# tdavchev/DESIRE

Hardware: AMD Instinct MI355X
Metric: agent-trajectory-samples/sec (K=20, T_pred=40) (higher is better)
Workload: dtype f32; 1 GPU; BASELINE configs[1]: SDD-like synthetic windows, 32 agent slots/window, K=20, T_obs=8/T_pred=40, H=128, L=128, fp32, posterior CVAE, IOC 1 refinement, social grid 4x4, scene grid 64x64x32; 512 windows/step/GPU; windows_per_gpu=512, rows_per_gpu=327680, parallelism=scene-sharded x1

## Files before the change

desire_amd/csrc/api.hip:

```cpp
#include "ctx.h"

#include <cmath>
#include <cstdio>
#include <cstdlib>
#include <cstring>

static thread_local std::string g_err;
int desire_fail(int code, const std::string& msg) { g_err = msg; return code; }

extern "C" const char* desire_last_error(void) { return g_err.c_str(); }
extern "C" int desire_version(void) { return 5; }
extern "C" int desire_dims_size(void) { return (int)sizeof(desire_dims); }
#ifndef DESIRE_SRC_HASH
#define DESIRE_SRC_HASH "unstamped"
#endif
extern "C" const char* desire_build_hash(void) { return DESIRE_SRC_HASH; }

int desire_upload(desire_ctx* h, const std::string& name, const std::vector<float>& v) {
    const size_t bytes = v.size() * sizeof(float);
    const DevBuf* b = h->dev.find(name.c_str());
    if (!b || b->bytes != bytes) {
        h->dev.release(name.c_str());
        if (h->dev.ensure(name.c_str(), bytes)) return -1;
    }
// ... 76 lines not shown
        return fail(DESIRE_ERR_ARG, "mno must divide 32 or be a multiple of 32 up to 256 (above 128: inference, step-wise IOC)");
    if (d.mno > 128 && d.bf16 == 1) return fail(DESIRE_ERR_ARG, "more than 128 agents per scene run the fp32 step-wise IOC (bf16 = 0, 2 or 3)");
    if (d.H != 16 && d.H != 32 && d.H != 64 && d.H != 128 && d.H != 256)
        return fail(DESIRE_ERR_ARG, "H must be 16, 32 (run zero-padded on the 64-wide tile), 64, 128 or 256");

    if (d.L % 8 || d.L < 8) return fail(DESIRE_ERR_ARG, "L must be a positive multiple of 8");
    if (d.C != 32 || d.E_v != 16) return fail(DESIRE_ERR_ARG, "C=32 and E_v=16 are the instantiated IOC widths in this round");
    if (d.n_scenes < 1 || d.K < 1 || d.T_obs < 1 || d.T_pred < 1 || d.n_grids < 1 || d.iters < 1 || d.Gh < 1 || d.Gw < 1)
        return fail(DESIRE_ERR_ARG, "sizes must be >= 1");
    if (d.grid_size < 1 || d.grid_size > 6) return fail(DESIRE_ERR_ARG, "grid_size must be 1..6 (6 x 6 = the paper's 36 bins)");
    if (d.grid_size > 4 && d.H == 256) return fail(DESIRE_ERR_ARG, "grid_size 5..6 needs H <= 128 (LDS budget of the IOC tile)");
    if (d.bf16 < 0 || d.bf16 > 3)
        return fail(DESIRE_ERR_ARG, "bf16 must be 0 (fp32 operands), 1 (bf16 operands), 2 (split-bf16 operands: hi + lo, three products) or 3 (three "
                                    "bf16 pieces, six products: fp32-class accuracy)");
    if (d.bn_mode < 0 || d.bn_mode > 2) return fail(DESIRE_ERR_ARG, "bn_mode must be 0 (frozen statistics), 1 (per-object statistics) or 2 (whole-batch statistics)");
    if (d.bn_mode && d.bf16 == 1) return fail(DESIRE_ERR_ARG, "batch statistics (bn_mode 1 / 2) run on fp32 operands (bf16 = 0 or 2)");
    if (d.bin_mode != 0 && d.bin_mode != 1) return fail(DESIRE_ERR_ARG, "bin_mode must be 0 (rectangular) or 1 (log-polar)");
    if (d.bin_mode == 1 && (d.grid_size < 3 || !(d.nb_h > 0.f) || !(d.nb_w > d.nb_h)))
        return fail(DESIRE_ERR_ARG, "log-polar bins: grid_size >= 3 and 0 < nb_h (inner radius) < nb_w (outer radius)");
    if (!(d.nb_w > 0.f) || !(d.nb_h > 0.f)) return fail(DESIRE_ERR_ARG, "nb_w/nb_h must be > 0");
    if (d.ref_compat != 0 && d.ref_compat != 1) return fail(DESIRE_ERR_ARG, "ref_compat must be 0 or 1");
    if (int rc = check_options(d)) return rc;
    if (d.ref_compat) {
        if (d.K != 1 || !d.posterior || d.bn_mode != 1 || d.bf16 || d.n_dec < 1 || d.H != 2 * d.T_obs || d.T_pred != d.T_obs)
            return fail(DESIRE_ERR_ARG, "ref_compat (the reference graph as written, model/model.py:116-311) needs K = 1 (one eps per object, "
                                        ":262-263), posterior = 1, bn_mode = 1, bf16 = 0, H == 2*T_obs (:286-289), T_pred == T_obs and n_dec >= 1 (:280 runs 7)");
    } else if (d.n_dec != 0) return fail(DESIRE_ERR_ARG, "n_dec belongs to ref_compat (0 otherwise)");
    return 0;
}

}

extern "C" int desire_set_option(desire_handle* h, const char* name, int32_t value) {
    if (!h || !name) return fail(DESIRE_ERR_ARG, "null argument");
    desire_dims d = h->d;
    const std::string nm(name);
    if (nm == "ioc_form") d.ioc_form = value;
    else if (nm == "ioc_split") d.ioc_split = value;
    else if (nm == "train_fp32_mask") d.train_fp32_mask = value;
    else if (nm == "flags") d.flags = value;
    else if (nm == "compact_host_counts") {
        h->cp_host_counts = value != 0;
        h->cp_pending = false; h->cp_enc = false;
        return DESIRE_OK;
    }
    else if (nm == "scene_grad") {
        if (value != 0 && value != 1) return fail(DESIRE_ERR_ARG, "scene_grad must be 0 or 1");
        h->scene_grad = value != 0;
        return scene_grad_on(h) && h->training ? scene_grad_setup(h) : DESIRE_OK;
    }
    else if (nm == "compact_min_rows") {
        if (value < 0) return fail(DESIRE_ERR_ARG, "compact_min_rows must be >= 0");
        h->ci_min_rows = value;
        return DESIRE_OK;
    }
    else return fail(DESIRE_ERR_ARG, "unknown option: " + nm + " (ioc_form, ioc_split, train_fp32_mask, flags, compact_min_rows, compact_host_counts, scene_grad)");
    if (int rc = check_options(d)) return rc;
    if (((d.flags ^ h->d.flags) & (DESIRE_FLAG_COMPACT_ROWS | DESIRE_FLAG_COMPACT_IOC)) ||
        ((d.flags & DESIRE_FLAG_COMPACT_IOC) && (d.ioc_form != h->d.ioc_form || d.train_fp32_mask != h->d.train_fp32_mask)))
        h->cp_pending = h->cp_enc = false;
    h->d = d;
    return DESIRE_OK;
}

extern "C" int desire_create(const desire_dims* dims, desire_handle** out) {
    if (!dims || !out) return fail(DESIRE_ERR_ARG, "null argument");
    if (int rc = check_dims(*dims)) return rc;
    int ndev = 0;
    if (hipGetDeviceCount(&ndev) != hipSuccess || ndev < 1)
        return fail(DESIRE_ERR_NODEV, "no HIP device: libdesire_hip has no CPU path");
    int dev = 0;
    HIPCHK(hipGetDevice(&dev));
    hipDeviceProp_t prop;
    HIPCHK(hipGetDeviceProperties(&prop, dev));
    if (std::strncmp(prop.gcnArchName, "gfx950", 6) != 0)
        return fail(DESIRE_ERR_NODEV, std::string("device is ") + prop.gcnArchName + ", kernels are built for gfx950 only");
    desire_ctx* h = new desire_ctx();
    h->d = *dims;
    h->Hl = dims->H;
    if (dims->H < 64) h->d.H = 64;
    h->A = dims->n_scenes * dims->mno;
    h->R = h->A * dims->K;
    h->V = dims->S * dims->S;
    h->B = dims->grid_size * dims->grid_size;
    h->E = dims->E_v + dims->C + h->d.H;
    pack::weight_shapes(h->d, h->d.H, h->V, h->B, h->want);
    pack::weight_shapes(h->d, h->Hl, h->V, h->B, h->want_user);
    if (h->Hl != h->d.H) embeddings(h);
    const desire_dims& d = h->d;
// ... 213 lines not shown
```

desire_amd/csrc/api_forward.hip:

```cpp
#include "ctx.h"

#include <cmath>
#include <cstdio>
#include <cstdlib>
#include <cstring>

bool compact_rows(const desire_ctx* h) { return (h->d.flags & DESIRE_FLAG_COMPACT_ROWS) != 0; }
bool compact_ioc(const desire_ctx* h) { return (h->d.flags & DESIRE_FLAG_COMPACT_IOC) && ioc_plan(h).fwd != IocFwd::STEPWISE; }
ClassLayout class_layout(const desire_ctx* h, bool pad, const int* counts) {
    const desire_dims& d = h->d;
    ClassLayout L;
    int cand[6], nc = 0;
    for (int m : {8, 10, 16, 32, 64, 96}) if (m < d.mno && (m != 10 || pad)) cand[nc++] = m;
    for (int i = nc > 3 ? nc - 3 : 0; i < nc; ++i) L.m[L.n++] = cand[i];
    L.m[L.n++] = d.mno;
    for (int i = L.n; i < 4; ++i) L.m[i] = d.mno;
    for (int c = 0; c < L.n; ++c) {
        IocView& v = L.c[c];
        v.cls = c; v.mno = L.m[c]; v.n_scenes = counts ? counts[c] : d.n_scenes;
        v.gpt = (v.mno <= 32 && 32 % v.mno) ? 32 / v.mno : 0; v.ngrp = v.n_scenes * d.K;
        v.R = v.gpt ? (long)((v.ngrp + v.gpt - 1) / v.gpt) * 32 : (long)v.ngrp * v.mno;
        v.agent_off = L.agents; v.row_off = L.rows; v.win_off = L.wins;
        L.agents += (size_t)v.n_scenes * v.mno; L.rows += (size_t)v.R; L.wins += (size_t)v.n_scenes;
    }
// ... 192 lines not shown
    const bool dyn = compact && compact_dyn(h);
    const int32_t* dynP = dyn ? Wt<const int32_t>(h, "cp_count") : nullptr;
    h->cp_last = compact;
    if (compact) {
        if (int rc = compact_wait(h, s)) return rc;
        int P = h->A;
        if (!dyn) { if (int rc = present_count(h, &P)) return rc; }
        h->cp_P = dyn ? -1 : P;
        R = P * d.K; mno = P;
        const size_t RT2 = (size_t)h->R * d.T_pred * 2;
        if (P == 0) {
            launch_fill_f32(W(h, "Y0"), RT2, 0.f, s); launch_fill_f32(dev_Yhat, RT2, 0.f, s);
            HIPCHK(hipGetLastError());
            return DESIRE_OK;
        }
        const int32_t* amap = Wt<const int32_t>(h, "cp_amap");
        Timer t(h, s, "compact_gather");
        if (!h->cp_enc) {
            launch_gather_agents(W(h, "HxHy"), W(h, "cp_HxHy"), amap, P, 2 * H, s, dynP);
            launch_gather_agents(W(h, "p_last"), W(h, "cp_plast"), amap, P, 2, s, dynP);
            if (d.posterior) launch_gather_agents(W(h, "params"), W(h, "cp_params"), amap, P, 2 * d.L, s, dynP);
        }
        HxS = W(h, "cp_HxHy"); plS = W(h, "cp_plast"); Yout = W(h, "cp_Y0");
    }
    if (compact) { Timer t(h, s, "reparam"); launch_reparam_c(W(h, "cp_params"), dev_eps, W(h, "z"), Wt<const int32_t>(h, "cp_amap"), mno, d.K, d.mno, d.L, d.posterior, s, dynP); }
    else { Timer t(h, s, "reparam"); launch_reparam(W(h, "params"), dev_eps, W(h, "z"), R, d.L, d.K, d.mno, d.posterior, s); }
    auto normd = [&](const char* layer, float* x, int P, int C, int sig) { batch_stats_act(h, layer, x, R, P, C, sig, s); };
    GemmArgs g{};
    g.A = W(h, "z"); g.lda = d.L; g.M = R; g.K = d.L; g.Bp = D4(h, "vae_dec/deconv1/W"); g.G = d.L / 8;
    g.NT = 64; g.out = W(h, "d1"); g.ldo = 2048; g.N = 2048;
    g.p0 = D(h, "vae_dec/deconv1/scale"); g.p1 = D(h, "vae_dec/deconv1/shift"); g.chmod = 128;
    int hintS = 0;
    if (dyn) hintS = count_hint(h);
    g.dyn = DynCount{dynP, d.K, hintS}; g.M_hint = hintS * d.K;
    const bool x6gen = ((d.bf16 == 3 && !h->training) || (d.bf16 == 2 && (!h->training || (train_x3_mask(h) & 8)))) && d.bn_mode == 0 && !d.ref_compat;
    if (d.bf16 == 1 && d.L <= 512 && !(d.L & 15)) { g.Bp = D4(h, "vae_dec/deconv1/W16"); Timer t(h, s, "deconv1"); launch_deconv1_bf16(g, s); }
    else if (x6gen && rows_x6_supported(d.L, 64)) { g.Bp = D4(h, "vae_dec/deconv1/W6"); Timer t(h, s, "deconv1"); launch_deconv1_x6(g, s); }
    else if (d.bn_mode != 0) {
        Timer t(h, s, "deconv1"); launch_gemm_rows(g, EPI_NONE, s);
        normd("vae_dec/deconv1", W(h, "d1"), 16, 128, 0);
    }
    else { Timer t(h, s, "deconv1"); launch_gemm_rows(g, EPI_SCALE_SHIFT_ELU, s); }
    ConvArgs c{};
    c.n = R; c.dyn = DynCount{dynP, d.K, hintS};
    const bool pobn = d.bn_mode != 0;
    if (pobn) c.mode = 3;
    c.in = W(h, "d1"); c.out = W(h, "d2"); c.Wp = D4(h, "vae_dec/deconv2/W");
    c.scale = D(h, "vae_dec/deconv2/scale"); c.shift = D(h, "vae_dec/deconv2/shift");
    if (d.bf16 == 1) { c.Wp = D4(h, "vae_dec/deconv2/W16"); Timer t(h, s, "deconv2"); launch_deconv2_bf16(c, s); }
    else if (x6gen) { c.Wp = D4(h, "vae_dec/deconv2/W6"); Timer t(h, s, "deconv2"); launch_deconv2_x6(c, s, (h->training && (d.flags & DESIRE_FLAG_TRAIN_FWD_3P)) ? 2 : 3); }
    else { Timer t(h, s, "deconv2"); launch_deconv2(c, s);
           if (pobn) normd("vae_dec/deconv2", W(h, "d2"), 64, 64, 0); }
    c.in = W(h, "d2"); c.out = W(h, "d3"); c.Wp = D4(h, "vae_dec/deconv3/W");
    c.scale = D(h, "vae_dec/deconv3/scale"); c.shift = D(h, "vae_dec/deconv3/shift");
    const bool fuse34 = d.bf16 == 1 && !(d.flags & DESIRE_FLAG_NO_FUSE34);
    if (fuse34) {
        c.Wp = D4(h, "vae_dec/deconv3/W16"); c.w_raw = D(h, "vae_dec/deconv4/W16"); c.out = W(h, "xhat");
        Timer t(h, s, "deconv34");
        launch_deconv34_bf16(c, D(h, "vae_dec/deconv4/scale"), D(h, "vae_dec/deconv4/shift"), s);
    } else {
        if (d.bf16 == 1) { c.Wp = D4(h, "vae_dec/deconv3/W16"); Timer t(h, s, "deconv3"); launch_deconv3_bf16(c, s); }
        else if (x6gen) { c.Wp = D4(h, "vae_dec/deconv3/W6"); Timer t(h, s, "deconv3"); launch_deconv3_x6(c, s, (h->training && (d.flags & DESIRE_FLAG_TRAIN_FWD_3P)) ? 2 : 3); }
        else { Timer t(h, s, "deconv3"); launch_deconv3(c, s);
               if (pobn) normd("vae_dec/deconv3", W(h, "d3"), 256, 32, 0); }
        c.in = W(h, "d3"); c.out = W(h, "xhat"); c.w_raw = D(h, "vae_dec/deconv4/raw");
        c.scale = D(h, "vae_dec/deconv4/scale"); c.shift = D(h, "vae_dec/deconv4/shift");
        { Timer t(h, s, "deconv4"); launch_deconv4(c, s);
          if (pobn) normd("vae_dec/deconv4", W(h, "xhat"), 1024, 1, 1); }
    }
    MaskArgs m{};
    m.xhat = W(h, "xhat"); m.R = R; m.V = h->V; m.H = H; m.Hl = h->Hl; m.K = d.K; m.mno = mno;
    m.Wp = D4(h, "mask/W"); m.bias = D(h, "mask/b"); m.Hx = HxS; m.ldhx = 2 * H; m.xz = W(h, "xz");
    m.dyn = DynCount{dynP, 1, hintS};
    if (h->training) m.sv_p = W(h, "mask_sv_p");
    if (d.bf16 == 1) { m.Wp = D4(h, "mask/W16"); Timer t(h, s, "mask_fc"); launch_mask_bf16(m, s); }
    else if (x6gen && (H == 64 || H == 128) && h->V % 128 == 0) { m.Wp = D4(h, "mask/W6"); Timer t(h, s, "mask_fc"); launch_mask_x6(m, s); }
    else { Timer t(h, s, "mask_fc"); launch_mask(m, s); }
    DecArgs a{};
    a.xz = W(h, "xz"); a.Hx = HxS; a.ldhx = 2 * H; a.p_last = plS;
    a.R = R; a.K = d.K; a.mno = mno; a.H = H; a.T = d.T_pred;
    a.Wxg = D4(h, "dec/Wxg"); a.Wxc = D4(h, "dec/Wxc"); a.Whg = D4(h, "dec/Whg"); a.Whc = D4(h, "dec/Whc");
    a.b_g = D(h, "dec/gb"); a.b_c = D(h, "dec/cb"); a.w_head = D(h, "head/w"); a.b_head = D(h, "head/b");
    a.Y = Yout; a.hdump = nullptr; a.dyn = DynCount{dynP, 1, hintS};
    if (d.ref_compat) { a.T = d.n_dec; a.hdump = W(h, "dec_states"); }
    if (h->training) { a.hdump = W(h, "dec_sv_h"); a.sv_r = W(h, "dec_sv_r"); a.sv_u = W(h, "dec_sv_u"); a.sv_c = W(h, "dec_sv_c"); }
    if (d.bf16 == 1) {
        a.Whg = D4(h, "dec/Whg16"); a.Whc = D4(h, "dec/Whc16");
        Timer t(h, s, "decoder"); launch_decoder_bf16(a, s);
    } else
    if (x6gen && decoder_x6_supported(H)) {
        a.Whg = D4(h, "dec/Whg6"); a.Whc = D4(h, "dec/Whc6");
        Timer t(h, s, "decoder"); launch_decoder_x6(a, s, (h->training && (d.flags & DESIRE_FLAG_TRAIN_FWD_3P)) ? 2 : 3);
    } else
    { Timer t(h, s, "decoder"); launch_decoder(a, s); }
    if (d.ref_compat)
        launch_copy_cols(dev_Yhat, W(h, "dec_states"), (size_t)R * d.n_dec, h->Hl, H, s);
    else if (compact) {
        Timer t(h, s, "compact_scatter");
        const size_t RT2 = (size_t)h->R * d.T_pred * 2;
        launch_fill_f32(W(h, "Y0"), RT2, 0.f, s); launch_fill_f32(dev_Yhat, RT2, 0.f, s);
        launch_scatter_rows(Yout, W(h, "Y0"), dev_Yhat, Wt<const int32_t>(h, "cp_amap"), mno, d.K, d.mno, d.T_pred * 2, s, dynP);
    } else
        launch_copy_f32(dev_Yhat, W(h, "Y0"), (size_t)R * d.T_pred * 2, s);
    HIPCHK(hipGetLastError());
    return DESIRE_OK;
}

int ioc_cluster_exchange(desire_ctx* h, size_t n_groups, bool reset_err, hipStream_t s) {
    if (int rc = ws_ensure(h, {{"hex", (size_t)2 * h->R * h->d.H * sizeof(float)}, {"grp_cnt", ((size_t)h->R / 32 + 1) * sizeof(int)}, {"ioc_err", sizeof(int)}})) return rc;
    HIPCHK(hipMemsetAsync(W(h, "grp_cnt"), 0, n_groups * sizeof(int), s));
    if (reset_err) HIPCHK(hipMemsetAsync(W(h, "ioc_err"), 0, sizeof(int), s));
    return DESIRE_OK;
}
int ioc_cluster_check(desire_ctx* h, hipStream_t s, const char* what) {
    int err = 0;
    HIPCHK(hipMemcpyAsync(&err, W(h, "ioc_err"), sizeof(int), hipMemcpyDeviceToHost, s));
    HIPCHK(hipStreamSynchronize(s));
    return err ? fail(DESIRE_ERR_HIP, std::string(what) + " hand-off timed out (workgroups of a group were not co-resident)") : DESIRE_OK;
}
#ifdef DESIRE_IOC_TIMING
void ioc_timing_report(const long long* dbg, const char* const* names, int n, hipStream_t s) {
    long long host[16];
    (void)hipStreamSynchronize(s); (void)hipMemcpy(host, dbg, n * sizeof(long long), hipMemcpyDeviceToHost);
    long long tot = 0; for (int k = 0; k < n; ++k) tot += host[k];
    for (int k = 0; k < n; ++k) fprintf(stderr, "[ioc timing] %-45s %12lld cyc  %5.1f%%\n", names[k], host[k], 100.0 * host[k] / (double)tot);
}
#endif

static int ioc_core(desire_handle* h, const IocView& v, hipStream_t s) {
    const desire_dims& d = h->d;
    if (h->training && d.bf16 == 1) return fail(DESIRE_ERR_STATE, "bf16 operands are inference-only");
    IocArgs a{};
    a.Y = v.Y; a.score = v.score; a.Hx = v.Hx; a.ldhx = 2 * d.H; a.p_last = v.p_last; a.valid = v.valid;
    a.R = (int)v.R; a.K = d.K; a.mno = v.mno; a.H = d.H; a.T = d.T_pred; a.iters = d.iters;
    a.C = d.C; a.Gh = d.Gh; a.Gw = d.Gw; a.E_v = d.E_v; a.G = d.grid_size; a.nb_w = d.nb_w; a.nb_h = d.nb_h;
    a.grids = h->grids; a.grid_of_scene = v.gos; a.bin_tab = d.bin_mode == 1 ? W(h, "bin_tab") : nullptr;
    a.w_vel = D(h, "ioc/vel_w"); a.b_vel = D(h, "ioc/vel_b");
    a.Wsoc = D4(h, "ioc/Wsoc"); a.b_soc = D(h, "ioc/soc_b"); a.Wsoc_c = D4(h, "ioc/Wsoc_c");
    a.Wg = D4(h, "ioc/Wg"); a.Wc = D4(h, "ioc/Wc"); a.b_g = D(h, "ioc/gb"); a.b_c = D(h, "ioc/cb");
    a.w_score = D(h, "ioc/score_w"); a.b_score = D(h, "ioc/score_b");
    a.Wreg = D4(h, "ioc/Wreg"); a.b_reg = D(h, "ioc/reg_b"); a.NTreg = (2 * d.T_pred + 31) / 32;
    a.variant = d.ioc_form; a.gpt = v.gpt; a.ngrp = v.ngrp; a.dyn = DynCount{v.dynN, 1, 0};
    const IocPlan p = ioc_plan(d, h->training, v.mno, v.gpt, v.R, [&](int n) { return ioc_bin_split_capacity(a, n); });
    if (!p.fp32_weights()) { a.Wsoc = D4(h, "ioc/Wsoc16"); a.Wg = D4(h, "ioc/Wg16"); a.Wc = D4(h, "ioc/Wc16"); a.Wreg = D4(h, "ioc/Wreg16"); }
    if (p.cluster()) {
        if (int rc = ioc_cluster_exchange(h, (size_t)v.R / v.mno, true, s)) return rc;
        a.hex = W(h, "hex"); a.grp_cnt = Wt<int>(h, "grp_cnt"); a.err = Wt<int>(h, "ioc_err");
    }
    if (p.nspl > 1) {
        const size_t tiles = ((size_t)v.R + 31) / 32, tiles_max = ((size_t)h->R + 31) / 32;
        if (int rc = ws_ensure(h, {{"hex_s", tiles_max * 2 * 4 * 32 * d.H * sizeof(float)}, {"cnt_s", tiles_max * sizeof(int)}})) return rc;
        if (!h->host_err) {
            if (hipHostMalloc(reinterpret_cast<void**>(&h->host_err), sizeof(int), hipHostMallocMapped) != hipSuccess || !h->host_err)
// ... 139 lines not shown
```

desire_amd/csrc/ctx.h:

```cpp
#pragma once
#include "../../include/desire_hip.h"
#include "ioc_plan.h"
#include "kernels.h"
#include "pack.h"
#include "workspace.h"

#include <hip/hip_runtime.h>

#include <cstring>
#include <functional>
#include <map>
#include <string>
#include <vector>

int desire_fail(int code, const std::string& msg);
#define fail desire_fail
#define HIPCHK(x)                                                                                   \
    do {                                                                                            \
        hipError_t e_ = (x);                                                                        \
        if (e_ != hipSuccess)                                                                       \
            return fail(DESIRE_ERR_HIP, std::string(#x) + ": " + hipGetErrorString(e_));            \
    } while (0)

inline int dev_malloc(void** p, size_t bytes) { return hipMalloc(p, bytes) == hipSuccess ? 0 : -1; }
inline void dev_free(void* p) { (void)hipFree(p); }

struct Prof { std::string name; hipEvent_t e0, e1; };

struct WSlot { size_t off; size_t n; };

struct EmbedAxis { std::vector<std::pair<int, int>> seg; };
struct Embed { EmbedAxis rows, cols; };

struct desire_ctx {
    desire_dims d;
    int Hl = 0;
    int A, R, V, B, E;
    std::map<std::string, size_t> want_user;
    std::map<std::string, Embed> emb;
    std::map<std::string, std::vector<float>> host_w;
    std::map<std::string, size_t> want;
    Workspace dev{dev_malloc, dev_free};
    Workspace ws{dev_malloc, dev_free};
    bool finalized = false;
    std::vector<void*> graphs;
    std::vector<float> bin_tab_host;
    const float* grids = nullptr;
    bool grids_set = false;
    bool profiling = false;
    void* peer_region = nullptr; size_t peer_bytes = 0; void* peer_base[8] = {nullptr, nullptr, nullptr, nullptr, nullptr, nullptr, nullptr, nullptr};
    bool peer_mapped[8] = {false, false, false, false, false, false, false, false}; int peer_rank = -1, peer_nranks = 0; bool peer_ready = false;
    int* peer_err = nullptr;
    float head_loss_w = 0.f;
    int* host_err = nullptr;
    int32_t* cp_host = nullptr; hipEvent_t cp_ev = nullptr; bool cp_pending = false; int cp_P = -1;
    int ci_cnt[4] = {0, 0, 0, 0}; bool ci_last = false; int ci_min_rows = 8192;
    bool cp_enc = false;
    bool cp_host_counts = false;
    bool cp_last = false;
    int32_t* bw_starts = nullptr; int32_t* bw_err = nullptr;
    std::vector<Prof> prof;
    std::vector<std::string> prof_name_store;
    bool training = false;
    std::map<std::string, WSlot> slots;
    size_t n_params = 0;
    const float* last_eps = nullptr;
    int adam_t = 0;
    int n_seg = 0;
    int n_seg16 = 0;
    bool scene_grad = false;
    const float* img = nullptr; bool img_set = false;
    bool img_stale = true;
};

struct Timer {
    desire_ctx* h; hipStream_t s; bool on; size_t idx = 0;
    Timer(desire_ctx* h_, hipStream_t s_, const char* name) : h(h_), s(s_), on(h_->profiling) {
        if (!on) return;
        Prof p; p.name = name;
        (void)hipEventCreate(&p.e0); (void)hipEventCreate(&p.e1);
        (void)hipEventRecord(p.e0, s);
        idx = h->prof.size();
        h->prof.push_back(p);
    }
    ~Timer() { if (on) (void)hipEventRecord(h->prof[idx].e1, s); }
};

inline int train_x3_mask(const desire_ctx* h) { return 15 & ~h->d.train_fp32_mask; }
inline int wgrad_pieces(const desire_ctx* h) { return (h->d.bf16 == 2 && (train_x3_mask(h) & 1)) ? 2 : 0; }
inline bool dgrad_split(const desire_ctx* h) { return h->d.bf16 == 2 && (train_x3_mask(h) & 2); }
// ... 42 lines not shown
```

desire_amd/csrc/kernels.h:

```cpp
#pragma once
#include <hip/hip_runtime.h>
#include <stdint.h>

#include "dyn_count.h"
#include "ioc_lds.h"

template <auto K>
inline const void* big_lds_kernel() {
    static const hipError_t once = hipFuncSetAttribute(reinterpret_cast<const void*>(K), hipFuncAttributeMaxDynamicSharedMemorySize, 160 * 1024);
    (void)once;
    return reinterpret_cast<const void*>(K);
}
template <auto K, class... Args>
inline void launch_big_lds(dim3 grid, dim3 block, size_t lds, hipStream_t s, const Args&... args) {
    (void)big_lds_kernel<K>();
    hipLaunchKernelGGL(K, grid, block, lds, s, args...);
}


enum { EPI_BIAS = 0, EPI_BIAS_RELU = 1, EPI_SCALE_SHIFT_ELU = 2, EPI_NONE = 3, EPI_ELUGRAD = 4, EPI_SIGGRAD = 5 };

struct GemmArgs {
    const float* A; int lda; int M; int K;
    const float4* Bp; int G; int NT;
    float* out; int ldo; int N;
    const float* p0; const float* p1; int chmod;
    const float* aux;
    DynCount dyn;
    int M_hint;
};
void launch_gemm_rows(const GemmArgs& a, int epi, hipStream_t s);

void launch_reparam(const float* params, const float* eps, float* z, int R, int L, int K, int mno,
                    int posterior, hipStream_t s);

struct MaskArgs {
    const float* xhat; int R; int V; int H; int K; int mno;
    int Hl;
    const float4* Wp; const float* bias; const float* Hx; int ldhx; float* xz;
    float* sv_p;
    DynCount dyn;
};
void launch_mask(const MaskArgs& a, hipStream_t s);
bool rows_x6_supported(int K, int NT);
void launch_deconv1_x6(const GemmArgs& a, hipStream_t s);
void launch_mask_x6(const MaskArgs& a, hipStream_t s);

struct ConvArgs {
    const float* in; float* out; int n;
    const float4* Wp; const float* w_raw;
    const float* scale; const float* shift;
    int mode; const float* yprev;
    DynCount dyn;
};
void launch_conv1(const ConvArgs& a, hipStream_t s);
void launch_conv2(const ConvArgs& a, hipStream_t s);
void launch_conv2_x3(const ConvArgs& a, hipStream_t s);
void launch_conv3_x3(const ConvArgs& a, hipStream_t s);
void launch_conv3(const ConvArgs& a, hipStream_t s);
void launch_deconv2(const ConvArgs& a, hipStream_t s);
void launch_deconv3(const ConvArgs& a, hipStream_t s);
void launch_deconv4(const ConvArgs& a, hipStream_t s);

struct EncArgs {
    const float* frames; int n_scenes; int T; int mno;
    float sx, sy; int H;
    const float* wx_g; const float* b_g;
    const float* wx_c; const float* b_c;
    const float4* Whg; const float4* Whc;
    float* out; int ldo;
    float* p_last;
    uint8_t* valid;
    float* sv_r; float* sv_u; float* sv_c; float* sv_h; float* sv_x;
    int n_roll; const float* w5; const float* b5;
// ... 209 lines not shown
```

desire_amd/csrc/kernels_gemm.hip:

```cpp
#include "common.h"
#include "kernels.h"

#define KC 256
#define LDA_C (KC + 4)

template <int EPI, int NTW, int MT = 2>
__global__ __launch_bounds__(DS_WG, 2) void k_gemm_rows(GemmArgs a) {
    constexpr int TMR = 32 * MT;
    extern __shared__ __attribute__((aligned(16))) float smem[];
    const int lane = lane_id(), w = wave_id(), tid = threadIdx.x;
    const int row0 = blockIdx.x * TMR;
    DYN_N(a, M, row0)
    f32x16 acc[NTW][MT];
#pragma unroll
    for (int j = 0; j < NTW; ++j)
#pragma unroll
        for (int m = 0; m < MT; ++m) acc[j][m] = zero16();
    const float* a_lane = smem + (lane & 31) * LDA_C + 4 * (lane >> 5);

    for (int k0 = 0; k0 < a.K; k0 += KC) {
        const int kc = min(KC, a.K - k0);
        const int q = kc >> 2;
        for (int i = tid; i < TMR * q; i += DS_WG) {
            const int r = i / q, c4 = i - r * q;
            const int row = row0 + r;
            float4 v = make_float4(0.f, 0.f, 0.f, 0.f);
            if (row < a.M) v = *reinterpret_cast<const float4*>(a.A + (size_t)row * a.lda + k0 + c4 * 4);
            *reinterpret_cast<float4*>(smem + r * LDA_C + c4 * 4) = v;
        }
        __syncthreads();
#pragma unroll
        for (int j = 0; j < NTW; ++j) {
            const int nt = (blockIdx.y * NTW + j) * 4 + w;
            if (nt < a.NT)
                mma_groups<MT>(acc[j], a_lane, LDA_C, a.Bp + ((size_t)nt * a.G + (k0 >> 3)) * 64 + lane, kc >> 3);
        }
        __syncthreads();
    }
#pragma unroll
    for (int j = 0; j < NTW; ++j) {
        const int nt = (blockIdx.y * NTW + j) * 4 + w;
        if (nt >= a.NT) continue;
        const int col = nt * 32 + (lane & 31);
        if (col >= a.N) continue;
        float p0 = 0.f, p1 = 0.f;
        if (EPI == EPI_SCALE_SHIFT_ELU) { const int ch = col % a.chmod; p0 = a.p0[ch]; p1 = a.p1[ch]; }
        else if (EPI == EPI_ELUGRAD || EPI == EPI_SIGGRAD) p0 = a.p0[col % a.chmod];
        else if (EPI != EPI_NONE) p0 = a.p0[col];
#pragma unroll
        for (int m = 0; m < MT; ++m)
#pragma unroll
            for (int i = 0; i < 16; ++i) {
                const int row = row0 + m * 32 + acc_row(i);
                if (row >= a.M) continue;
                float v = acc[j][m][i];
                if (EPI == EPI_BIAS) v = v + p0;
                else if (EPI == EPI_BIAS_RELU) v = fmaxf(v + p0, 0.f);
                else if (EPI == EPI_SCALE_SHIFT_ELU) v = eluf_(v * p0 + p1);
                else if (EPI == EPI_ELUGRAD) { const float y = a.aux[(size_t)row * a.ldo + col]; v = v * (y > 0.f ? 1.0f : y + 1.0f) * p0; }
                else if (EPI == EPI_SIGGRAD) { const float y = a.aux[(size_t)row * a.ldo + col]; v = v * y * (1.0f - y) * p0; }
                a.out[(size_t)row * a.ldo + col] = v;
            }
    }
}

template <int NTW, int MT>
static void launch_gemm_rows_n(const GemmArgs& a, int epi, hipStream_t s) {
    constexpr int TMR = 32 * MT;
    dim3 grid((a.M + TMR - 1) / TMR, (a.NT + 4 * NTW - 1) / (4 * NTW));
    const size_t lds = TMR * LDA_C * sizeof(float);
    if (epi == EPI_NONE) launch_big_lds<k_gemm_rows<EPI_NONE, NTW, MT>>(grid, dim3(DS_WG), lds, s, a);
    else if (epi == EPI_ELUGRAD) launch_big_lds<k_gemm_rows<EPI_ELUGRAD, NTW, MT>>(grid, dim3(DS_WG), lds, s, a);
    else if (epi == EPI_SIGGRAD) launch_big_lds<k_gemm_rows<EPI_SIGGRAD, NTW, MT>>(grid, dim3(DS_WG), lds, s, a);
    else if (epi == EPI_BIAS) launch_big_lds<k_gemm_rows<EPI_BIAS, NTW, MT>>(grid, dim3(DS_WG), lds, s, a);
    else if (epi == EPI_BIAS_RELU) launch_big_lds<k_gemm_rows<EPI_BIAS_RELU, NTW, MT>>(grid, dim3(DS_WG), lds, s, a);
    else launch_big_lds<k_gemm_rows<EPI_SCALE_SHIFT_ELU, NTW, MT>>(grid, dim3(DS_WG), lds, s, a);
}
void launch_gemm_rows(const GemmArgs& a, int epi, hipStream_t s) {
    const int Msel = (a.dyn.cnt && a.M_hint > 0) ? a.M_hint : a.M;
    const long wgs = (long)((Msel + DS_TM - 1) / DS_TM) * ((a.NT + 15) / 16);
    if (wgs < 128) launch_gemm_rows_n<1, 1>(a, epi, s); else launch_gemm_rows_n<4, 2>(a, epi, s);
}

__global__ void k_reparam(const float* __restrict__ params, const float* __restrict__ eps,
                          float* __restrict__ z, int R, int L, int K, int mno, int posterior) {
    const int i = blockIdx.x * blockDim.x + threadIdx.x;
    if (i >= R * L) return;
    const int r = i / L, l = i - r * L;
    float e = eps[i];
    if (posterior) {
        const int a = agent_of_row(r, K, mno);
        const float mu = params[(size_t)a * 2 * L + l], ls = params[(size_t)a * 2 * L + L + l];
        e = mu + sqrtf(expf(ls)) * e;
    }
    z[i] = e;
}

void launch_reparam(const float* params, const float* eps, float* z, int R, int L, int K, int mno,
                    int posterior, hipStream_t s) {
    const int n = R * L;
    hipLaunchKernelGGL(k_reparam, dim3((n + 255) / 256), dim3(256), 0, s, params, eps, z, R, L, K, mno, posterior);
}

__global__ __launch_bounds__(DS_WG) void k_mask(MaskArgs a) {
    extern __shared__ __attribute__((aligned(16))) float smem[];
    const int lane = lane_id(), w = wave_id(), tid = threadIdx.x;
    const int row0 = blockIdx.x * DS_TM;
    DYN_P(a, row0)
    const int NT = a.H >> 5;
    f32x16 acc[2][2] = {{zero16(), zero16()}, {zero16(), zero16()}};
    const float* a_lane = smem + (lane & 31) * LDA_C + 4 * (lane >> 5);
    const int G = a.V >> 3;
    for (int k0 = 0; k0 < a.V; k0 += KC) {
        const int q = KC >> 2;
        for (int i = tid; i < DS_TM * q; i += DS_WG) {
            const int r = i / q, c4 = i - r * q;
            const int row = row0 + r;
            float4 v = make_float4(0.f, 0.f, 0.f, 0.f);
            if (row < a.R) v = *reinterpret_cast<const float4*>(a.xhat + (size_t)row * a.V + k0 + c4 * 4);
            *reinterpret_cast<float4*>(smem + r * LDA_C + c4 * 4) = v;
        }
        __syncthreads();
#pragma unroll
        for (int j = 0; j < 2; ++j) {
            const int nt = w + 4 * j;
            if (nt < NT) mma_groups<2>(acc[j], a_lane, LDA_C, a.Wp + ((size_t)nt * G + (k0 >> 3)) * 64 + lane, KC >> 3);
        }
        __syncthreads();
    }
    const int LDT = a.H + 4;
#pragma unroll
    for (int j = 0; j < 2; ++j) {
        const int nt = w + 4 * j;
        if (nt >= NT) continue;
        const int col = nt * 32 + (lane & 31);
        const float b = a.bias[col];
#pragma unroll
        for (int m = 0; m < 2; ++m)
#pragma unroll
            for (int i = 0; i < 16; ++i) {
                const float pv = fmaxf(acc[j][m][i] + b, 0.f);
                smem[(m * 32 + acc_row(i)) * LDT + col] = pv;
                if (a.sv_p && row0 + m * 32 + acc_row(i) < a.R) a.sv_p[(size_t)(row0 + m * 32 + acc_row(i)) * a.H + col] = pv;
            }
    }
    __syncthreads();
    const int r = tid >> 2, q4 = tid & 3;
    const int row = row0 + r;
    const int nv = a.H >> 4;
    float4* trow = reinterpret_cast<float4*>(smem + r * LDT);
    float mx = -3.0e38f;
    for (int j = 0; j < nv; ++j) { const float4 v = trow[4 * j + q4]; mx = fmaxf(mx, fmaxf(fmaxf(v.x, v.y), fmaxf(v.z, v.w))); }
    mx = fmaxf(mx, __shfl_xor(mx, 1));
    mx = fmaxf(mx, __shfl_xor(mx, 2));
    float sum = 0.f;
    for (int j = 0; j < nv; ++j) {
        float4 v = trow[4 * j + q4];
        v.x = expf(v.x - mx); v.y = expf(v.y - mx); v.z = expf(v.z - mx); v.w = expf(v.w - mx);
        trow[4 * j + q4] = v;
        const int c0 = 16 * j + 4 * q4;
        sum += (c0 < a.Hl ? v.x : 0.f) + (c0 + 1 < a.Hl ? v.y : 0.f) + (c0 + 2 < a.Hl ? v.z : 0.f) + (c0 + 3 < a.Hl ? v.w : 0.f);
    }
    sum += __shfl_xor(sum, 1);
    sum += __shfl_xor(sum, 2);
    if (row < a.R) {
        const int ag = agent_of_row(row, a.K, a.mno);
        const float inv = 1.0f / sum;
        const float4* hx = reinterpret_cast<const float4*>(a.Hx + (size_t)ag * a.ldhx);
        float4* xz = reinterpret_cast<float4*>(a.xz + (size_t)row * a.H);
        for (int j = 0; j < nv; ++j) {
            const float4 e = trow[4 * j + q4], hv = hx[4 * j + q4];
            xz[4 * j + q4] = make_float4(e.x * inv * hv.x, e.y * inv * hv.y, e.z * inv * hv.z, e.w * inv * hv.w);
        }
    }
}

void launch_mask(const MaskArgs& a, hipStream_t s) {
    const size_t lds = DS_TM * LDA_C * sizeof(float);
    launch_big_lds<k_mask>(dim3((a.R + DS_TM - 1) / DS_TM), dim3(DS_WG), lds, s, a);
}
```

Baseline: 2.415 million samples/s.

## Add register-streaming deconv1 GEMM and double-buffered pipelined mask kernel

Adds k_deconv1_stream, which keeps each wave's A rows in registers and streams B fragments with double-buffered loads, dropping the LDS staging and barriers for the scale-shift-ELU deconv1 GEMM. It also adds k_mask_pipe, which double-buffers xhat chunks in LDS and prefetches the next chunk into registers, so each chunk needs one barrier and loads overlap the MFMA work. A row_gemm_generic option and DESIRE_ROW_TIMING instrumentation let the old paths and per-phase timings be selected. The trade-offs are higher register pressure (launch bounds of 2 waves per SIMD), repeated A loads across N splits, and a larger LDS footprint.

```diff
diff --git a/desire_amd/csrc/api.hip b/desire_amd/csrc/api.hip
--- a/desire_amd/csrc/api.hip
+++ b/desire_amd/csrc/api.hip
@@ -132,9 +132,14 @@
 }
 
 extern "C" int desire_set_option(desire_handle* h, const char* name, int32_t value) {
-    if (!h || !name) return fail(DESIRE_ERR_ARG, "null argument");
+    if (!name) return fail(DESIRE_ERR_ARG, "null argument");
+    const std::string nm(name);
+    static const char* const known[] = {"ioc_form", "ioc_split", "train_fp32_mask", "flags", "compact_min_rows", "compact_host_counts", "row_gemm_generic", "scene_grad"};
+    bool is_known = false;
+    for (const char* k : known) is_known = is_known || nm == k;
+    if (!is_known) return fail(DESIRE_ERR_ARG, "unknown option: " + nm + " (ioc_form, ioc_split, train_fp32_mask, flags, compact_min_rows, compact_host_counts, row_gemm_generic, scene_grad)");
+    if (!h) return fail(DESIRE_ERR_ARG, "null argument");
     desire_dims d = h->d;
-    const std::string nm(name);
     if (nm == "ioc_form") d.ioc_form = value;
     else if (nm == "ioc_split") d.ioc_split = value;
     else if (nm == "train_fp32_mask") d.train_fp32_mask = value;
@@ -144,6 +149,11 @@
         h->cp_pending = false; h->cp_enc = false;
         return DESIRE_OK;
     }
+    else if (nm == "row_gemm_generic") {
+        if (value != 0 && value != 1) return fail(DESIRE_ERR_ARG, "row_gemm_generic must be 0 or 1");
+        h->row_gemm_generic = value != 0;
+        return DESIRE_OK;
+    }
     else if (nm == "scene_grad") {
         if (value != 0 && value != 1) return fail(DESIRE_ERR_ARG, "scene_grad must be 0 or 1");
         h->scene_grad = value != 0;
@@ -154,7 +164,7 @@
         h->ci_min_rows = value;
         return DESIRE_OK;
     }
-    else return fail(DESIRE_ERR_ARG, "unknown option: " + nm + " (ioc_form, ioc_split, train_fp32_mask, flags, compact_min_rows, compact_host_counts, scene_grad)");
+    else return fail(DESIRE_ERR_ARG, "unknown option: " + nm);
     if (int rc = check_options(d)) return rc;
     if (((d.flags ^ h->d.flags) & (DESIRE_FLAG_COMPACT_ROWS | DESIRE_FLAG_COMPACT_IOC)) ||
         ((d.flags & DESIRE_FLAG_COMPACT_IOC) && (d.ioc_form != h->d.ioc_form || d.train_fp32_mask != h->d.train_fp32_mask)))
diff --git a/desire_amd/csrc/api_forward.hip b/desire_amd/csrc/api_forward.hip
--- a/desire_amd/csrc/api_forward.hip
+++ b/desire_amd/csrc/api_forward.hip
@@ -248,7 +248,7 @@
     g.p0 = D(h, "vae_dec/deconv1/scale"); g.p1 = D(h, "vae_dec/deconv1/shift"); g.chmod = 128;
     int hintS = 0;
     if (dyn) hintS = count_hint(h);
-    g.dyn = DynCount{dynP, d.K, hintS}; g.M_hint = hintS * d.K;
+    g.dyn = DynCount{dynP, d.K, hintS}; g.M_hint = hintS * d.K; g.generic = h->row_gemm_generic;
     const bool x6gen = ((d.bf16 == 3 && !h->training) || (d.bf16 == 2 && (!h->training || (train_x3_mask(h) & 8)))) && d.bn_mode == 0 && !d.ref_compat;
     if (d.bf16 == 1 && d.L <= 512 && !(d.L & 15)) { g.Bp = D4(h, "vae_dec/deconv1/W16"); Timer t(h, s, "deconv1"); launch_deconv1_bf16(g, s); }
     else if (x6gen && rows_x6_supported(d.L, 64)) { g.Bp = D4(h, "vae_dec/deconv1/W6"); Timer t(h, s, "deconv1"); launch_deconv1_x6(g, s); }
@@ -256,7 +256,14 @@
         Timer t(h, s, "deconv1"); launch_gemm_rows(g, EPI_NONE, s);
         normd("vae_dec/deconv1", W(h, "d1"), 16, 128, 0);
     }
-    else { Timer t(h, s, "deconv1"); launch_gemm_rows(g, EPI_SCALE_SHIFT_ELU, s); }
+    else {
+#ifdef DESIRE_ROW_TIMING
+        if (int rc = ws_ensure(h, {{"dbg_rows", 16 * sizeof(long long)}})) return rc;
+        g.dbg = Wt<long long>(h, "dbg_rows");
+        (void)hipMemsetAsync(g.dbg, 0, 16 * sizeof(long long), s);
+#endif
+        Timer t(h, s, "deconv1"); launch_gemm_rows(g, EPI_SCALE_SHIFT_ELU, s);
+    }
     ConvArgs c{};
     c.n = R; c.dyn = DynCount{dynP, d.K, hintS};
     const bool pobn = d.bn_mode != 0;
@@ -287,11 +294,27 @@
     MaskArgs m{};
     m.xhat = W(h, "xhat"); m.R = R; m.V = h->V; m.H = H; m.Hl = h->Hl; m.K = d.K; m.mno = mno;
     m.Wp = D4(h, "mask/W"); m.bias = D(h, "mask/b"); m.Hx = HxS; m.ldhx = 2 * H; m.xz = W(h, "xz");
-    m.dyn = DynCount{dynP, 1, hintS};
+    m.dyn = DynCount{dynP, 1, hintS}; m.generic = h->row_gemm_generic;
     if (h->training) m.sv_p = W(h, "mask_sv_p");
     if (d.bf16 == 1) { m.Wp = D4(h, "mask/W16"); Timer t(h, s, "mask_fc"); launch_mask_bf16(m, s); }
     else if (x6gen && (H == 64 || H == 128) && h->V % 128 == 0) { m.Wp = D4(h, "mask/W6"); Timer t(h, s, "mask_fc"); launch_mask_x6(m, s); }
-    else { Timer t(h, s, "mask_fc"); launch_mask(m, s); }
+    else {
+#ifdef DESIRE_ROW_TIMING
+        if (int rc = ws_ensure(h, {{"dbg_rows", 16 * sizeof(long long)}})) return rc;
+        m.dbg = Wt<long long>(h, "dbg_rows") + 8;
+#endif
+        Timer t(h, s, "mask_fc"); launch_mask(m, s);
+    }
+#ifdef DESIRE_ROW_TIMING
+    if (d.bf16 == 0 && d.bn_mode == 0) {
+        const char* nd[8] = {"deconv1 generic: stage A -> LDS | stream: load B + contract a tile", "deconv1 generic: barrier 1 | stream: epilogue + stores of a tile",
+                             "deconv1 generic: contraction", "deconv1 generic: barrier 2", "deconv1 generic: epilogue + stores", "-", "-", "-"};
+        const char* nm[8] = {"mask generic: stage chunk -> LDS | pipe: weight head + issue next chunk's loads", "mask: barrier (pipe: the only one per chunk)",
+                             "mask: contraction", "mask generic: barrier 2 | pipe: registers -> other buffer", "mask: relu tile + barrier", "mask: softmax * Hx", "-", "-"};
+        ioc_timing_report(Wt<long long>(h, "dbg_rows"), nd, 8, s);
+        ioc_timing_report(Wt<long long>(h, "dbg_rows") + 8, nm, 8, s);
+    }
+#endif
     DecArgs a{};
     a.xz = W(h, "xz"); a.Hx = HxS; a.ldhx = 2 * H; a.p_last = plS;
     a.R = R; a.K = d.K; a.mno = mno; a.H = H; a.T = d.T_pred;
@@ -334,7 +357,7 @@
     HIPCHK(hipStreamSynchronize(s));
     return err ? fail(DESIRE_ERR_HIP, std::string(what) + " hand-off timed out (workgroups of a group were not co-resident)") : DESIRE_OK;
 }
-#ifdef DESIRE_IOC_TIMING
+#if defined(DESIRE_IOC_TIMING) || defined(DESIRE_ROW_TIMING)
 void ioc_timing_report(const long long* dbg, const char* const* names, int n, hipStream_t s) {
     long long host[16];
     (void)hipStreamSynchronize(s); (void)hipMemcpy(host, dbg, n * sizeof(long long), hipMemcpyDeviceToHost);
diff --git a/desire_amd/csrc/ctx.h b/desire_amd/csrc/ctx.h
--- a/desire_amd/csrc/ctx.h
+++ b/desire_amd/csrc/ctx.h
@@ -56,6 +56,7 @@
     int32_t* cp_host = nullptr; hipEvent_t cp_ev = nullptr; bool cp_pending = false; int cp_P = -1;
     int ci_cnt[4] = {0, 0, 0, 0}; bool ci_last = false; int ci_min_rows = 8192;
     bool cp_enc = false;
+    bool row_gemm_generic = false;
     bool cp_host_counts = false;
     bool cp_last = false;
     int32_t* bw_starts = nullptr; int32_t* bw_err = nullptr;
diff --git a/desire_amd/csrc/kernels.h b/desire_amd/csrc/kernels.h
--- a/desire_amd/csrc/kernels.h
+++ b/desire_amd/csrc/kernels.h
@@ -28,6 +28,8 @@
     const float* aux;
     DynCount dyn;
     int M_hint;
+    long long* dbg;
+    int generic;
 };
 void launch_gemm_rows(const GemmArgs& a, int epi, hipStream_t s);
 
@@ -40,6 +42,8 @@
     const float4* Wp; const float* bias; const float* Hx; int ldhx; float* xz;
     float* sv_p;
     DynCount dyn;
+    long long* dbg;
+    int generic;
 };
 void launch_mask(const MaskArgs& a, hipStream_t s);
 bool rows_x6_supported(int K, int NT);
diff --git a/desire_amd/csrc/kernels_gemm.hip b/desire_amd/csrc/kernels_gemm.hip
--- a/desire_amd/csrc/kernels_gemm.hip
+++ b/desire_amd/csrc/kernels_gemm.hip
@@ -2,6 +2,16 @@
 #include "kernels.h"
 
 #define KC 256
+
+#ifdef DESIRE_ROW_TIMING
+#define ROW_TIMING_BEGIN long long tacc[8] = {0, 0, 0, 0, 0, 0, 0, 0}; long long tprev = clock64();
+#define ROW_TICK(k) { const long long now_ = clock64(); tacc[k] += now_ - tprev; tprev = now_; }
+#define ROW_TIMING_END(a) if ((a).dbg && blockIdx.x == gridDim.x / 2 && blockIdx.y == 0 && threadIdx.x == 0) for (int k_ = 0; k_ < 8; ++k_) (a).dbg[k_] = tacc[k_];
+#else
+#define ROW_TIMING_BEGIN
+#define ROW_TICK(k)
+#define ROW_TIMING_END(a)
+#endif
 #define LDA_C (KC + 4)
 
 template <int EPI, int NTW, int MT = 2>
@@ -11,6 +21,7 @@
     const int lane = lane_id(), w = wave_id(), tid = threadIdx.x;
     const int row0 = blockIdx.x * TMR;
     DYN_N(a, M, row0)
+    ROW_TIMING_BEGIN
     f32x16 acc[NTW][MT];
 #pragma unroll
     for (int j = 0; j < NTW; ++j)
@@ -28,14 +39,18 @@
             if (row < a.M) v = *reinterpret_cast<const float4*>(a.A + (size_t)row * a.lda + k0 + c4 * 4);
             *reinterpret_cast<float4*>(smem + r * LDA_C + c4 * 4) = v;
         }
-        __syncthreads();
+        ROW_TICK(0)
+        __syncthreads();
+        ROW_TICK(1)
 #pragma unroll
         for (int j = 0; j < NTW; ++j) {
             const int nt = (blockIdx.y * NTW + j) * 4 + w;
             if (nt < a.NT)
                 mma_groups<MT>(acc[j], a_lane, LDA_C, a.Bp + ((size_t)nt * a.G + (k0 >> 3)) * 64 + lane, kc >> 3);
         }
-        __syncthreads();
+        ROW_TICK(2)
+        __syncthreads();
+        ROW_TICK(3)
     }
 #pragma unroll
     for (int j = 0; j < NTW; ++j) {
@@ -62,6 +77,8 @@
                 a.out[(size_t)row * a.ldo + col] = v;
             }
     }
+    ROW_TICK(4)
+    ROW_TIMING_END(a)
 }
 
 template <int NTW, int MT>
@@ -76,10 +93,100 @@
     else if (epi == EPI_BIAS_RELU) launch_big_lds<k_gemm_rows<EPI_BIAS_RELU, NTW, MT>>(grid, dim3(DS_WG), lds, s, a);
     else launch_big_lds<k_gemm_rows<EPI_SCALE_SHIFT_ELU, NTW, MT>>(grid, dim3(DS_WG), lds, s, a);
 }
+template <int G, int MT>
+__device__ __forceinline__ void stream_mma4(f32x16 (&acc)[MT], const float4 (&af)[MT][G], int g, const float4 (&b)[4]) {
+#pragma unroll
+    for (int j = 0; j < 4; ++j)
+#pragma unroll
+        for (int m = 0; m < MT; ++m) {
+            const float4 av = af[m][g + j];
+            acc[m] = mfma32(b[j].x, av.x, acc[m]);
+            acc[m] = mfma32(b[j].y, av.y, acc[m]);
+            acc[m] = mfma32(b[j].z, av.z, acc[m]);
+            acc[m] = mfma32(b[j].w, av.w, acc[m]);
+        }
+}
+template <int G, int MT>
+__global__ __launch_bounds__(DS_WG, 2) void k_deconv1_stream(GemmArgs a, int ntw) {
+    const int lane = lane_id(), w = wave_id(), hi = lane >> 5, c = lane & 31;
+    const int row0 = (blockIdx.x * 4 + w) * (32 * MT);
+    DYN_N(a, M, row0)
+    if (row0 >= a.M) return;
+    ROW_TIMING_BEGIN
+    float4 af[MT][G];
+#pragma unroll
+    for (int m = 0; m < MT; ++m) {
+        const int row = min(row0 + m * 32 + c, a.M - 1);
+        const float* src = a.A + (size_t)row * a.lda + 4 * hi;
+#pragma unroll
+        for (int g = 0; g < G; ++g) af[m][g] = *reinterpret_cast<const float4*>(src + g * 8);
+    }
+    const int nt0 = blockIdx.y * ntw, nt1 = min(nt0 + ntw, a.NT);
+    const float4* b_lane = a.Bp + (size_t)nt0 * G * 64 + lane;
+    const int g_last = (nt1 - nt0) * G - 4;
+    const unsigned loff = (unsigned)c * (unsigned)a.ldo + 4u * hi;
+    float4 b0[4], b1[4];
+    load_b4(b0, b_lane, 0);
+    int fg = 0;
+#pragma clang loop unroll(disable)
+    for (int nt = nt0; nt < nt1; ++nt, fg += G) {
+        f32x16 acc[MT];
+#pragma unroll
+        for (int m = 0; m < MT; ++m) acc[m] = zero16();
+#pragma unroll
+        for (int p = 0; p < G / 8; ++p) {
+            load_b4(b1, b_lane, fg + 8 * p + 4);
+            __builtin_amdgcn_sched_barrier(0);
+            stream_mma4<G, MT>(acc, af, 8 * p, b0);
+            __builtin_amdgcn_sched_barrier(0);
+            load_b4(b0, b_lane, min(fg + 8 * p + 8, g_last));
+            __builtin_amdgcn_sched_barrier(0);
+            stream_mma4<G, MT>(acc, af, 8 * p + 4, b1);
+            __builtin_amdgcn_sched_barrier(0);
+        }
+        ROW_TICK(0)
+        const int ch0 = (nt * 32) % a.chmod + 4 * hi;
+        float4 s4[4], t4[4];
+#pragma unroll
+        for (int q = 0; q < 4; ++q) {
+            s4[q] = *reinterpret_cast<const float4*>(a.p0 + ch0 + 8 * q);
+            t4[q] = *reinterpret_cast<const float4*>(a.p1 + ch0 + 8 * q);
+        }
+#pragma unroll
+        for (int m = 0; m < MT; ++m) {
+            if (row0 + m * 32 + c >= a.M) continue;
+            float* o = a.out + (size_t)(row0 + m * 32) * a.ldo + nt * 32;
+#pragma unroll
+            for (int q = 0; q < 4; ++q) {
+                float4 v;
+                v.x = eluf_(acc[m][4 * q] * s4[q].x + t4[q].x);
+                v.y = eluf_(acc[m][4 * q + 1] * s4[q].y + t4[q].y);
+                v.z = eluf_(acc[m][4 * q + 2] * s4[q].z + t4[q].z);
+                v.w = eluf_(acc[m][4 * q + 3] * s4[q].w + t4[q].w);
+                *reinterpret_cast<float4*>(o + loff + 8 * q) = v;
+            }
+        }
+        ROW_TICK(1)
+    }
+    ROW_TIMING_END(a)
+}
+static bool deconv1_stream_ok(const GemmArgs& a) {
+    return (a.K == 64 || a.K == 128) && a.G * 8 == a.K && !(a.lda & 3) && !(a.ldo & 3) && a.N == a.NT * 32 && a.chmod > 0 && !(a.chmod & 31);
+}
+template <int G>
+static void launch_deconv1_stream(const GemmArgs& a, int rows, hipStream_t s) {
+    const long rwg = (rows + 255) / 256;
+    int ntw = a.NT;
+    while (ntw > 4 && rwg * ((a.NT + ntw - 1) / ntw) < 512) ntw = (ntw + 1) / 2;
+    dim3 grid((a.M + 255) / 256, (a.NT + ntw - 1) / ntw);
+    hipLaunchKernelGGL((k_deconv1_stream<G, 2>), grid, dim3(DS_WG), 0, s, a, ntw);
+}
 void launch_gemm_rows(const GemmArgs& a, int epi, hipStream_t s) {
     const int Msel = (a.dyn.cnt && a.M_hint > 0) ? a.M_hint : a.M;
     const long wgs = (long)((Msel + DS_TM - 1) / DS_TM) * ((a.NT + 15) / 16);
-    if (wgs < 128) launch_gemm_rows_n<1, 1>(a, epi, s); else launch_gemm_rows_n<4, 2>(a, epi, s);
+    if (wgs < 128) launch_gemm_rows_n<1, 1>(a, epi, s);
+    else if (epi == EPI_SCALE_SHIFT_ELU && !a.generic && deconv1_stream_ok(a)) { if (a.K == 128) launch_deconv1_stream<16>(a, Msel, s); else launch_deconv1_stream<8>(a, Msel, s); }
+    else launch_gemm_rows_n<4, 2>(a, epi, s);
 }
 
 __global__ void k_reparam(const float* __restrict__ params, const float* __restrict__ eps,
@@ -102,49 +209,7 @@
     hipLaunchKernelGGL(k_reparam, dim3((n + 255) / 256), dim3(256), 0, s, params, eps, z, R, L, K, mno, posterior);
 }
 
-__global__ __launch_bounds__(DS_WG) void k_mask(MaskArgs a) {
-    extern __shared__ __attribute__((aligned(16))) float smem[];
-    const int lane = lane_id(), w = wave_id(), tid = threadIdx.x;
-    const int row0 = blockIdx.x * DS_TM;
-    DYN_P(a, row0)
-    const int NT = a.H >> 5;
-    f32x16 acc[2][2] = {{zero16(), zero16()}, {zero16(), zero16()}};
-    const float* a_lane = smem + (lane & 31) * LDA_C + 4 * (lane >> 5);
-    const int G = a.V >> 3;
-    for (int k0 = 0; k0 < a.V; k0 += KC) {
-        const int q = KC >> 2;
-        for (int i = tid; i < DS_TM * q; i += DS_WG) {
-            const int r = i / q, c4 = i - r * q;
-            const int row = row0 + r;
-            float4 v = make_float4(0.f, 0.f, 0.f, 0.f);
-            if (row < a.R) v = *reinterpret_cast<const float4*>(a.xhat + (size_t)row * a.V + k0 + c4 * 4);
-            *reinterpret_cast<float4*>(smem + r * LDA_C + c4 * 4) = v;
-        }
-        __syncthreads();
-#pragma unroll
-        for (int j = 0; j < 2; ++j) {
-            const int nt = w + 4 * j;
-            if (nt < NT) mma_groups<2>(acc[j], a_lane, LDA_C, a.Wp + ((size_t)nt * G + (k0 >> 3)) * 64 + lane, KC >> 3);
-        }
-        __syncthreads();
-    }
-    const int LDT = a.H + 4;
-#pragma unroll
-    for (int j = 0; j < 2; ++j) {
-        const int nt = w + 4 * j;
-        if (nt >= NT) continue;
-        const int col = nt * 32 + (lane & 31);
-        const float b = a.bias[col];
-#pragma unroll
-        for (int m = 0; m < 2; ++m)
-#pragma unroll
-            for (int i = 0; i < 16; ++i) {
-                const float pv = fmaxf(acc[j][m][i] + b, 0.f);
-                smem[(m * 32 + acc_row(i)) * LDT + col] = pv;
-                if (a.sv_p && row0 + m * 32 + acc_row(i) < a.R) a.sv_p[(size_t)(row0 + m * 32 + acc_row(i)) * a.H + col] = pv;
-            }
-    }
-    __syncthreads();
+__device__ __forceinline__ void mask_softmax_rows(const MaskArgs& a, float* smem, int LDT, int row0, int tid) {
     const int r = tid >> 2, q4 = tid & 3;
     const int row = row0 + r;
     const int nv = a.H >> 4;
@@ -175,7 +240,141 @@
     }
 }
 
+__global__ __launch_bounds__(DS_WG) void k_mask(MaskArgs a) {
+    extern __shared__ __attribute__((aligned(16))) float smem[];
+    const int lane = lane_id(), w = wave_id(), tid = threadIdx.x;
+    const int row0 = blockIdx.x * DS_TM;
+    DYN_P(a, row0)
+    const int NT = a.H >> 5;
+    ROW_TIMING_BEGIN
+    f32x16 acc[2][2] = {{zero16(), zero16()}, {zero16(), zero16()}};
+    const float* a_lane = smem + (lane & 31) * LDA_C + 4 * (lane >> 5);
+    const int G = a.V >> 3;
+    for (int k0 = 0; k0 < a.V; k0 += KC) {
+        const int q = KC >> 2;
+        for (int i = tid; i < DS_TM * q; i += DS_WG) {
+            const int r = i / q, c4 = i - r * q;
+            const int row = row0 + r;
+            float4 v = make_float4(0.f, 0.f, 0.f, 0.f);
+            if (row < a.R) v = *reinterpret_cast<const float4*>(a.xhat + (size_t)row * a.V + k0 + c4 * 4);
+            *reinterpret_cast<float4*>(smem + r * LDA_C + c4 * 4) = v;
+        }
+        ROW_TICK(0)
+        __syncthreads();
+        ROW_TICK(1)
+#pragma unroll
+        for (int j = 0; j < 2; ++j) {
+            const int nt = w + 4 * j;
+            if (nt < NT) mma_groups<2>(acc[j], a_lane, LDA_C, a.Wp + ((size_t)nt * G + (k0 >> 3)) * 64 + lane, KC >> 3);
+        }
+        ROW_TICK(2)
+        __syncthreads();
+        ROW_TICK(3)
+    }
+    const int LDT = a.H + 4;
+#pragma unroll
+    for (int j = 0; j < 2; ++j) {
+        const int nt = w + 4 * j;
+        if (nt >= NT) continue;
+        const int col = nt * 32 + (lane & 31);
+        const float b = a.bias[col];
+#pragma unroll
+        for (int m = 0; m < 2; ++m)
+#pragma unroll
+            for (int i = 0; i < 16; ++i) {
+                const float pv = fmaxf(acc[j][m][i] + b, 0.f);
+                smem[(m * 32 + acc_row(i)) * LDT + col] = pv;
+                if (a.sv_p && row0 + m * 32 + acc_row(i) < a.R) a.sv_p[(size_t)(row0 + m * 32 + acc_row(i)) * a.H + col] = pv;
+            }
+    }
+    __syncthreads();
+    ROW_TICK(4)
+    mask_softmax_rows(a, smem, LDT, row0, tid);
+    ROW_TICK(5)
+    ROW_TIMING_END(a)
+}
+
+#define KC2 128
+#define LDA_C2 (KC2 + 4)
+template <int NJ>
+__global__ __launch_bounds__(DS_WG, 2) void k_mask_pipe(MaskArgs a) {
+    extern __shared__ __attribute__((aligned(16))) float smem[];
+    const int lane = lane_id(), w = wave_id(), tid = threadIdx.x;
+    const int row0 = blockIdx.x * DS_TM;
+    DYN_P(a, row0)
+    const int NT = a.H >> 5;
+    ROW_TIMING_BEGIN
+    f32x16 acc[NJ][2];
+#pragma unroll
+    for (int j = 0; j < NJ; ++j) { acc[j][0] = zero16(); acc[j][1] = zero16(); }
+    const int G = a.V >> 3, nchunk = a.V / KC2;
+    constexpr int NLD = DS_TM * (KC2 / 4) / DS_WG;
+    const int sr = tid >> 5, sc4 = tid & 31;
+    float4 st[NLD];
+    auto fetch = [&](int k0) {
+#pragma unroll
+        for (int t = 0; t < NLD; ++t) {
+            const int row = row0 + sr + 8 * t;
+            st[t] = make_float4(0.f, 0.f, 0.f, 0.f);
+            if (row < a.R) st[t] = *reinterpret_cast<const float4*>(a.xhat + (size_t)row * a.V + k0 + sc4 * 4);
+        }
+    };
+    auto put = [&](float* buf) {
+#pragma unroll
+        for (int t = 0; t < NLD; ++t) *reinterpret_cast<float4*>(buf + (sr + 8 * t) * LDA_C2 + sc4 * 4) = st[t];
+    };
+    fetch(0);
+    put(smem);
+    const bool live = w < NT;
+    for (int c = 0; c < nchunk; ++c) {
+        float* cur = smem + (c & 1) * (DS_TM * LDA_C2);
+        const float* ap[2] = {cur + (lane & 31) * LDA_C2 + 4 * (lane >> 5), cur + (32 + (lane & 31)) * LDA_C2 + 4 * (lane >> 5)};
+        const float4* b_lane = a.Wp + ((size_t)w * G + c * (KC2 >> 3)) * 64 + lane;
+        MmaHead hd;
+        if (live) mma_begin(hd, b_lane, KC2 >> 3);
+        if (c + 1 < nchunk) fetch((c + 1) * KC2);
+        ROW_TICK(0)
+        __syncthreads();
+        ROW_TICK(1)
+        if (live) mma_run<2>(acc[0], ap, b_lane, KC2 >> 3, hd);
+        if (NJ == 2) mma_groups_ptr<2>(acc[NJ - 1], ap, a.Wp + ((size_t)(w + 4) * G + c * (KC2 >> 3)) * 64 + lane, KC2 >> 3);
+        ROW_TICK(2)
+        if (c + 1 < nchunk) put(smem + ((c + 1) & 1) * (DS_TM * LDA_C2));
+        ROW_TICK(3)
+    }
+    __syncthreads();
+    const int LDT = a.H + 4;
+#pragma unroll
+    for (int j = 0; j < NJ; ++j) {
+        const int nt = w + 4 * j;
+        if (nt >= NT) continue;
+        const int col = nt * 32 + (lane & 31);
+        const float b = a.bias[col];
+#pragma unroll
+        for (int m = 0; m < 2; ++m)
+#pragma unroll
+            for (int i = 0; i < 16; ++i) {
+                const float pv = fmaxf(acc[j][m][i] + b, 0.f);
+                smem[(m * 32 + acc_row(i)) * LDT + col] = pv;
+                if (a.sv_p && row0 + m * 32 + acc_row(i) < a.R) a.sv_p[(size_t)(row0 + m * 32 + acc_row(i)) * a.H + col] = pv;
+            }
+    }
+    __syncthreads();
+    ROW_TICK(4)
+    mask_softmax_rows(a, smem, LDT, row0, tid);
+    ROW_TICK(5)
+    ROW_TIMING_END(a)
+}
+
 void launch_mask(const MaskArgs& a, hipStream_t s) {
+    const dim3 grid((a.R + DS_TM - 1) / DS_TM);
+    if (!a.generic && a.V % KC2 == 0 && (a.H == 64 || a.H == 128 || a.H == 256)) {
+        const size_t tile = (size_t)DS_TM * (a.H + 4), bufs = 2 * (size_t)DS_TM * LDA_C2;
+        const size_t lds = (tile > bufs ? tile : bufs) * sizeof(float);
+        if (a.H == 256) launch_big_lds<k_mask_pipe<2>>(grid, dim3(DS_WG), lds, s, a);
+        else launch_big_lds<k_mask_pipe<1>>(grid, dim3(DS_WG), lds, s, a);
+        return;
+    }
     const size_t lds = DS_TM * LDA_C * sizeof(float);
-    launch_big_lds<k_mask>(dim3((a.R + DS_TM - 1) / DS_TM), dim3(DS_WG), lds, s, a);
-}
+    launch_big_lds<k_mask>(grid, dim3(DS_WG), lds, s, a);
+}
```

Measured after the change: 2.427 million samples/s, median of 6. No clear change (+0.5%).
